# JokerYan/MS-GS

Measured on AMD Instinct MI355X. Metric: Mpixels/s fwd+bwd @1080p, 1M Gaussians; fraction of HBM roofline, higher is better.
Workload: dtype f32

## Files before the change

### ms-gs_amd/csrc/sort.hip

```cpp
#include "msgs_internal.h"

#include <algorithm>

namespace msgs {

namespace {

__device__ __forceinline__ uint32_t wave_inclusive_scan(uint32_t v, int lane) {
#pragma unroll
    for (int off = 1; off < 64; off <<= 1) {
        const uint32_t n = (uint32_t)__shfl_up((int)v, off);
        if (lane >= off) v += n;
    }
    return v;
}

__device__ __forceinline__ uint32_t block_exclusive_scan(uint32_t v, uint32_t* s_wave , uint32_t* total) {
    const int lane = threadIdx.x & 63, w = threadIdx.x >> 6;
    const uint32_t inc = wave_inclusive_scan(v, lane);
    if (lane == 63) s_wave[w] = inc;
    __syncthreads();
    uint32_t base = 0;
#pragma unroll
    for (int k = 0; k < 4; ++k) {
        const uint32_t t = s_wave[k];
        if (k < w) base += t;
    }
    *total = s_wave[0] + s_wave[1] + s_wave[2] + s_wave[3];
    __syncthreads();
    return base + inc - v;
}

__device__ __forceinline__ void scan_load_items(const uint32_t* in, int64_t base, int64_t n, uint32_t v[SCAN_ITEMS]) {
    static_assert(SCAN_ITEMS % 4 == 0, "uint4 runs");
    if (base + SCAN_ITEMS <= n && (reinterpret_cast<uintptr_t>(in + base) & 15) == 0) {
#pragma unroll
        for (int q = 0; q < SCAN_ITEMS / 4; ++q) {
            const uint4 a = *reinterpret_cast<const uint4*>(in + base + 4 * q);
            v[4 * q] = a.x; v[4 * q + 1] = a.y; v[4 * q + 2] = a.z; v[4 * q + 3] = a.w;
        }
    } else {
#pragma unroll
        for (int k = 0; k < SCAN_ITEMS; ++k) v[k] = base + k < n ? in[base + k] : 0u;
    }
}
__device__ __forceinline__ void scan_store_items(uint32_t* out, int64_t base, int64_t n, const uint32_t v[SCAN_ITEMS]) {
    if (base + SCAN_ITEMS <= n && (reinterpret_cast<uintptr_t>(out + base) & 15) == 0) {
#pragma unroll
        for (int q = 0; q < SCAN_ITEMS / 4; ++q)
            *reinterpret_cast<uint4*>(out + base + 4 * q) = make_uint4(v[4 * q], v[4 * q + 1], v[4 * q + 2], v[4 * q + 3]);
    } else {
#pragma unroll
        for (int k = 0; k < SCAN_ITEMS; ++k) if (base + k < n) out[base + k] = v[k];
    }
}

__global__ __launch_bounds__(SCAN_THREADS) void scan_reduce_kernel(const uint32_t* __restrict__ in,
                                                                   const uint32_t* __restrict__ gather,
                                                                   int64_t n, uint64_t* __restrict__ partials,
                                                                   uint32_t* __restrict__ staged,
                                                                   const uint32_t* __restrict__ n_ptr, uint32_t in_mask,
                                                                   uint32_t* __restrict__ side_out, uint32_t* __restrict__ side_flag) {
    __shared__ uint32_t s_wave[4];
    if (n_ptr) n = (int64_t)*n_ptr;
    if (side_flag && blockIdx.x == 0 && threadIdx.x == 0) *side_flag = side_out ? 1u : 0u;
    const int64_t base = (int64_t)blockIdx.x * SCAN_CHUNK + (int64_t)threadIdx.x * SCAN_ITEMS;
    uint32_t v[SCAN_ITEMS];
    if (gather) {
        uint32_t g[SCAN_ITEMS];
        scan_load_items(gather, base, n, g);
#pragma unroll
        for (int k = 0; k < SCAN_ITEMS; ++k) v[k] = base + k < n ? in[g[k]] : 0u;
        if (side_out) {
#pragma unroll
            for (int k = 0; k < SCAN_ITEMS; ++k) g[k] = v[k] >> TILE_COUNT_BITS;
            scan_store_items(side_out, base, n, g);
        }
#pragma unroll
        for (int k = 0; k < SCAN_ITEMS; ++k) v[k] &= in_mask;
        if (staged) scan_store_items(staged, base, n, v);
    } else {
        scan_load_items(in, base, n, v);
    }
    uint32_t sum = 0;
#pragma unroll
    for (int k = 0; k < SCAN_ITEMS; ++k) sum += v[k];
    uint32_t total;
    block_exclusive_scan(sum, s_wave, &total);
    if (threadIdx.x == 0) partials[blockIdx.x] = total;
}

__global__ __launch_bounds__(SCAN_THREADS) void scan_apply_fused_kernel(const uint32_t* in, uint32_t* out, int64_t n,
                                                                        const uint64_t* __restrict__ partials, int64_t nb,
                                                                        const uint32_t* __restrict__ n_ptr,
                                                                        uint64_t* __restrict__ total_out,
                                                                        uint64_t* __restrict__ status,
                                                                        volatile uint64_t* host, uint64_t ticket,
                                                                        uint32_t* __restrict__ clamped_total, uint64_t clamp,
                                                                        const uint32_t* __restrict__ extra,
                                                                        uint32_t* __restrict__ zero_word,
                                                                        uint32_t* __restrict__ overflow_flag) {
    __shared__ uint32_t s_wave[4];
    __shared__ uint64_t s_sum[4];
    if (n_ptr) n = (int64_t)*n_ptr;
    const int lane = threadIdx.x & 63, w = threadIdx.x >> 6;
    const int64_t chunk0 = (int64_t)blockIdx.x * SCAN_CHUNK;
    if (blockIdx.x != 0 && chunk0 >= n) return;
    const int64_t upto = blockIdx.x == 0 ? nb : (int64_t)blockIdx.x;
    uint64_t acc = 0;
    for (int64_t q = threadIdx.x; q < upto; q += SCAN_THREADS) acc += partials[q];
    for (int off = 32; off > 0; off >>= 1)
        acc += ((uint64_t)(uint32_t)__shfl_xor((int)(uint32_t)(acc >> 32), off) << 32) | (uint32_t)__shfl_xor((int)(uint32_t)acc, off);
    if (lane == 0) s_sum[w] = acc;
    __syncthreads();
    const uint64_t sum = s_sum[0] + s_sum[1] + s_sum[2] + s_sum[3];
    uint64_t base = sum;
    if (blockIdx.x == 0) {
        base = 0;
        if (threadIdx.x == 0) {
            if (total_out) *total_out = sum;
            if (zero_word) *zero_word = 0u;
            if (clamped_total) *clamped_total = (uint32_t)(sum < clamp ? sum : clamp);
            if (overflow_flag && sum > clamp) *overflow_flag = 1u;
            const uint64_t info = extra ? ((uint64_t)extra[0] | ((uint64_t)extra[1] << 32)) : 0ull;
            if (status) { status[0] = sum; status[1] = 0; status[2] = info; }
            if (host) {
                host[0] = sum;
                host[1] = 0;
                host[3] = info;
                __threadfence_system();
                host[2] = ticket;
            }
        }
        if (chunk0 >= n) return;
    }
    const int64_t tb = chunk0 + (int64_t)threadIdx.x * SCAN_ITEMS;
    uint32_t v[SCAN_ITEMS];
    scan_load_items(in, tb, n, v);
    uint32_t tsum = 0;
#pragma unroll
    for (int k = 0; k < SCAN_ITEMS; ++k) tsum += v[k];
    uint32_t total;
    uint32_t run = block_exclusive_scan(tsum, s_wave, &total) + (uint32_t)base;
#pragma unroll
    for (int k = 0; k < SCAN_ITEMS; ++k) {
        const uint32_t x = v[k];
        v[k] = run;
        run += x;
    }
    scan_store_items(out, tb, n, v);
}

template <int ITEMS = SORT_ITEMS>
__device__ __forceinline__ int64_t elem_index(int64_t chunk_base, int w, int r, int lane) {
    return chunk_base + (int64_t)w * (64 * ITEMS) + r * 64 + lane;
}

template <int ITEMS, bool DROP = false, typename KeyT = uint32_t>
__global__ __launch_bounds__(SORT_THREADS) void radix_hist_kernel(const KeyT* __restrict__ keys, int64_t n,
                                                                  int shift, uint32_t mask, int64_t nblocks,
                                                                  uint32_t* __restrict__ hist,
                                                                  uint32_t* __restrict__ gsum, int gsize, int ngroups,
                                                                  const uint32_t* __restrict__ n_ptr = nullptr) {
    __shared__ uint32_t s_hist[256];
    const int64_t chunk_base = (int64_t)blockIdx.x * (SORT_THREADS * ITEMS);
    if (n_ptr) {
        n = (int64_t)*n_ptr;
        if (chunk_base >= n) return;
    }
    s_hist[threadIdx.x] = 0;
    __syncthreads();
    const int lane = threadIdx.x & 63, w = threadIdx.x >> 6;
    constexpr int KPV = 16 / (int)sizeof(KeyT);
    if (ITEMS % KPV == 0 && chunk_base + (int64_t)SORT_THREADS * ITEMS <= n) {
        const uint4* kv = reinterpret_cast<const uint4*>(keys + chunk_base);
#pragma unroll
        for (int r = 0; r < ITEMS / KPV; ++r) {
            const uint4 v = kv[r * SORT_THREADS + threadIdx.x];
            const uint32_t w4[4] = {v.x, v.y, v.z, v.w};
#pragma unroll
            for (int j = 0; j < KPV; ++j) {
                const uint32_t k = sizeof(KeyT) == 4 ? w4[j] : ((w4[j >> 1] >> ((j & 1) * 16)) & 0xFFFFu);
                if (!DROP || k != 0xFFFFFFFFu) atomicAdd(&s_hist[(k >> shift) & mask], 1u);
            }
        }
    } else {
#pragma unroll
        for (int r = 0; r < ITEMS; ++r) {
            const int64_t i = elem_index<ITEMS>(chunk_base, w, r, lane);
            if (i < n) {
                const uint32_t k = (uint32_t)keys[i];
                if (!DROP || k != 0xFFFFFFFFu) atomicAdd(&s_hist[(k >> shift) & mask], 1u);
            }
        }
    }
    __syncthreads();
    const uint32_t c = s_hist[threadIdx.x];
    hist[(int64_t)blockIdx.x * 256 + threadIdx.x] = c;
    if (c) atomicAdd(&gsum[(int64_t)(blockIdx.x / gsize) * 256 + threadIdx.x], c);
}

__global__ __launch_bounds__(256) void group_scan_kernel(uint32_t* __restrict__ gsum, int ngroups,
                                                         uint32_t* __restrict__ hist, int gsize, int64_t nblocks,
                                                         const uint32_t* __restrict__ n_ptr, int chunk) {
    if (n_ptr) {
        const int64_t n = (int64_t)*n_ptr;
        nblocks = (n + chunk - 1) / chunk;
        ngroups = (int)((nblocks + gsize - 1) / gsize);
        if ((int)blockIdx.x > ngroups) return;
        if (nblocks == 0) return;
    }
    const int d = threadIdx.x;
    if ((int)blockIdx.x < ngroups) {
        const int64_t first = (int64_t)blockIdx.x * gsize;
        const int rows = (int)min((int64_t)gsize, nblocks - first);
        uint32_t* q = hist + first * 256 + d;
        uint32_t run = 0;
#pragma unroll 8
        for (int k = 0; k < rows; ++k) {
            const uint32_t v = q[(int64_t)k * 256];
            q[(int64_t)k * 256] = run;
            run += v;
        }
        return;
    }
    __shared__ uint32_t s_wv[4];
    uint32_t tot = 0;
#pragma unroll 8
    for (int k = 0; k < ngroups; ++k) tot += gsum[(int64_t)k * 256 + d];
    uint32_t dummy;
    uint32_t run = block_exclusive_scan(tot, s_wv, &dummy);
#pragma unroll 8
    for (int k = 0; k < ngroups; ++k) {
        uint32_t* q = &gsum[(int64_t)k * 256 + d];
        const uint32_t v = *q;
        *q = run;
        run += v;
    }
}

template <int ITEMS, bool DROP = false, typename KeyT = uint32_t>
__global__ __launch_bounds__(SORT_THREADS) void radix_scatter_kernel(const KeyT* __restrict__ keys_in,
                                                                     const uint32_t* __restrict__ vals_in,
                                                                     KeyT* __restrict__ keys_out,
                                                                     uint32_t* __restrict__ vals_out, int64_t n,
                                                                     int shift, uint32_t mask, int64_t nblocks,
                                                                     const uint32_t* __restrict__ hist_scanned,
                                                                     const uint32_t* __restrict__ gsum, int gsize,
                                                                     int ngroups, bool gsum_is_base = false,
                                                                     const uint32_t* __restrict__ n_ptr = nullptr,
                                                                     uint32_t* __restrict__ n_out = nullptr) {
    __shared__ uint32_t s_cnt[4][256];
    __shared__ uint32_t s_wave[4];
    const int lane = threadIdx.x & 63, w = threadIdx.x >> 6;
    const int64_t chunk_base = (int64_t)blockIdx.x * (SORT_THREADS * ITEMS);
    if (n_ptr) {
        n = (int64_t)*n_ptr;
        if (chunk_base >= n) return;
    }
#pragma unroll
    for (int k = 0; k < 4; ++k) s_cnt[k][threadIdx.x] = 0;
    __syncthreads();

    uint32_t key[ITEMS], val[ITEMS], rank[ITEMS];
    const uint64_t lt_mask = (1ull << lane) - 1ull;
#pragma unroll
    for (int r = 0; r < ITEMS; ++r) {
        const int64_t i = elem_index<ITEMS>(chunk_base, w, r, lane);
        key[r] = i < n ? (uint32_t)keys_in[i] : 0xFFFFFFFFu;
        const bool valid = i < n && (!DROP || key[r] != 0xFFFFFFFFu);
        val[r] = valid ? (vals_in ? vals_in[i] : (uint32_t)i) : 0u;
        const uint32_t d = (key[r] >> shift) & mask;
        uint64_t peers = __ballot(valid);
#pragma unroll
        for (int b = 0; b < 8; ++b) {
            const uint64_t m = __ballot((d >> b) & 1u);
            peers &= ((d >> b) & 1u) ? m : ~m;
        }
        const uint32_t prev = s_cnt[w][d];
        const uint32_t before = (uint32_t)__popcll(peers & lt_mask);
        rank[r] = prev + before;
        if (valid && before == 0) s_cnt[w][d] = prev + (uint32_t)__popcll(peers);
    }
    __syncthreads();
    uint32_t gbase;
    {
        const uint32_t d = threadIdx.x;
        if (gsum_is_base) {
            const int g = blockIdx.x / gsize;
            gbase = gsum[(int64_t)g * 256 + d] + hist_scanned[(int64_t)blockIdx.x * 256 + d];
        } else {
            const int g = blockIdx.x / gsize;
            uint32_t tot = 0, before = 0;
#pragma unroll 8
            for (int k = 0; k < ngroups; ++k) {
                const uint32_t v = gsum[(int64_t)k * 256 + d];
                tot += v;
                before += k < g ? v : 0u;
            }
            const int nin = (int)(blockIdx.x - (int64_t)g * gsize);
            const uint32_t* hrow = hist_scanned + ((int64_t)g * gsize) * 256 + d;
#pragma unroll 8
            for (int k = 0; k < nin; ++k) before += hrow[(int64_t)k * 256];
            uint32_t total;
            gbase = block_exclusive_scan(tot, s_wave, &total) + before;
            if (n_out && blockIdx.x == 0 && threadIdx.x == 0) *n_out = total;
        }
    }
    __shared__ uint32_t s_key[SORT_THREADS * ITEMS], s_val[SORT_THREADS * ITEMS], s_delta[256];
    uint32_t nkept;
    {
        const uint32_t d = threadIdx.x;
        uint32_t c[4], ltot = 0;
#pragma unroll
        for (int k = 0; k < 4; ++k) { c[k] = s_cnt[k][d]; ltot += c[k]; }
        const uint32_t lbase = block_exclusive_scan(ltot, s_wave, &nkept);
        uint32_t run = lbase;
#pragma unroll
        for (int k = 0; k < 4; ++k) { s_cnt[k][d] = run; run += c[k]; }
        s_delta[d] = gbase - lbase;
    }
    __syncthreads();
#pragma unroll
    for (int r = 0; r < ITEMS; ++r) {
        const int64_t i = elem_index<ITEMS>(chunk_base, w, r, lane);
        if (i < n && (!DROP || key[r] != 0xFFFFFFFFu)) {
            const uint32_t lp = s_cnt[w][(key[r] >> shift) & mask] + rank[r];
            s_key[lp] = key[r];
            s_val[lp] = val[r];
        }
    }
    __syncthreads();
    const int nvalid = DROP ? (int)nkept : (int)min((int64_t)(SORT_THREADS * ITEMS), n - chunk_base);
#pragma unroll
    for (int r = 0; r < ITEMS; ++r) {
        const int j = r * SORT_THREADS + threadIdx.x;
        if (j < nvalid) {
            const uint32_t k = s_key[j];
            const uint32_t pos = (uint32_t)j + s_delta[(k >> shift) & mask];
            keys_out[pos] = (KeyT)k;
            vals_out[pos] = s_val[j];
        }
    }
}

}

hipError_t exclusive_scan_u32(const uint32_t* in, const uint32_t* gather, uint32_t* out, int64_t n,
                              uint64_t* partials, uint64_t* total, hipStream_t s, uint64_t* status,
                              uint64_t* host_mapped, uint64_t ticket, const uint32_t* n_ptr, uint32_t* clamped_total,
                              uint64_t clamp, const uint32_t* extra, uint32_t* zero_word, uint32_t* overflow_flag,
                              uint32_t in_mask, uint32_t* side_out, uint32_t* side_flag) {
    if ((in_mask != 0xFFFFFFFFu || side_out) && gather == nullptr) return hipErrorInvalidValue;
    if (n <= 0) {
        hipLaunchKernelGGL(scan_apply_fused_kernel, dim3(1), dim3(SCAN_THREADS), 0, s, in, out, (int64_t)0,
                           (const uint64_t*)partials, (int64_t)0, (const uint32_t*)nullptr, total, status,
                           (volatile uint64_t*)host_mapped, ticket, clamped_total, clamp, extra, zero_word, overflow_flag);
        return hipGetLastError();
    }
    if (gather != nullptr && out == in) return hipErrorInvalidValue;
    const int64_t nb = scan_blocks(n);
    const bool stage = gather != nullptr;
    hipLaunchKernelGGL(scan_reduce_kernel, dim3((unsigned)nb), dim3(SCAN_THREADS), 0, s, in, gather, n, partials,
                       stage ? out : (uint32_t*)nullptr, n_ptr, in_mask, side_out, side_flag);
    hipLaunchKernelGGL(scan_apply_fused_kernel, dim3((unsigned)nb), dim3(SCAN_THREADS), 0, s,
                       stage ? (const uint32_t*)out : in, out, n, (const uint64_t*)partials, nb, n_ptr, total, status,
                       (volatile uint64_t*)host_mapped, ticket, clamped_total, clamp, extra, zero_word, overflow_flag);
    return hipGetLastError();
}

namespace {
__global__ __launch_bounds__(256) void zero_kernel(uint32_t* __restrict__ p, size_t n_words) {
    const size_t n4 = n_words >> 2;
    uint4* p4 = reinterpret_cast<uint4*>(p);
    for (size_t i = (size_t)blockIdx.x * blockDim.x + threadIdx.x; i < n4; i += (size_t)gridDim.x * blockDim.x)
        p4[i] = make_uint4(0u, 0u, 0u, 0u);
    if (blockIdx.x == 0 && threadIdx.x < (n_words & 3)) p[(n4 << 2) + threadIdx.x] = 0u;
}
}

hipError_t launch_zero(void* ptr, size_t bytes, hipStream_t s) {
    if (bytes == 0) return hipSuccess;
    if ((reinterpret_cast<uintptr_t>(ptr) & 15) || (bytes & 3)) return hipMemsetAsync(ptr, 0, bytes, s);
    const size_t words = bytes >> 2;
    size_t blocks = (words / 4 + 255) / 256;
    if (blocks < 1) blocks = 1;
    if (blocks > 2048) blocks = 2048;
    hipLaunchKernelGGL(zero_kernel, dim3((unsigned)blocks), dim3(256), 0, s, (uint32_t*)ptr, words);
    return hipGetLastError();
}

static int passes_for(int begin_bit, int end_bit) {
    const int passes = (end_bit - begin_bit + 7) / 8;
    return passes < 1 ? 1 : passes;
}
typedef SortGeom GroupGeom;

bool radix_sort_supports_device_count(int64_t n, int begin_bit, int end_bit) {
    return n > 0 && passes_for(begin_bit, end_bit) <= 4;
}

bool radix_sort_keys16_ok(int64_t n, int begin_bit, int end_bit) {
    return end_bit <= 16 && radix_sort_supports_device_count(n, begin_bit, end_bit);
}

bool radix_sort_zero_region(int64_t n, int begin_bit, int end_bit, char* scratch, uint32_t** ptr, size_t* words) {
    if (n <= 0) return false;
    const int passes = passes_for(begin_bit, end_bit);
    if (passes > 4) return false;
    const GroupGeom G(n);
    const SortScratch L(n);
    *ptr = reinterpret_cast<uint32_t*>(scratch + L.hist) + (size_t)256 * G.nb;
    *words = G.zero_words(passes);
    return true;
}

namespace {
__global__ void store_u32_kernel(uint32_t* p, uint32_t v) { *p = v; }

template <int ITEMS, typename KeyT>
void launch_pass(const KeyT* src_k, const uint32_t* src_v, KeyT* dst_k, uint32_t* dst_v, int64_t n, int shift, uint32_t mask,
                 const GroupGeom& G, uint32_t* hist, uint32_t* gs, bool drop, const uint32_t* n_ptr, uint32_t* n_out,
                 hipStream_t s) {
    const dim3 grid((unsigned)G.nb), block(SORT_THREADS);
    if (drop) {
        hipLaunchKernelGGL((radix_hist_kernel<ITEMS, true, KeyT>), grid, block, 0, s, src_k, n, shift, mask, G.nb, hist, gs, G.gsize,
                           G.ngroups, (const uint32_t*)nullptr);
        hipLaunchKernelGGL((radix_scatter_kernel<ITEMS, true, KeyT>), grid, block, 0, s, src_k, src_v, dst_k, dst_v, n, shift,
                           mask, G.nb, hist, gs, G.gsize, G.ngroups, false, (const uint32_t*)nullptr, n_out);
        return;
    }
    hipLaunchKernelGGL((radix_hist_kernel<ITEMS, false, KeyT>), grid, block, 0, s, src_k, n, shift, mask, G.nb, hist, gs, G.gsize,
                       G.ngroups, n_ptr);
    if (G.scanned)
        hipLaunchKernelGGL(group_scan_kernel, dim3((unsigned)G.ngroups + 1), dim3(256), 0, s, gs, G.ngroups, hist, G.gsize, G.nb, n_ptr,
                           SORT_THREADS * ITEMS);
    hipLaunchKernelGGL((radix_scatter_kernel<ITEMS, false, KeyT>), grid, block, 0, s, src_k, src_v, dst_k, dst_v, n, shift, mask,
                       G.nb, hist, gs, G.gsize, G.ngroups, G.scanned, n_ptr, (uint32_t*)nullptr);
}

template <typename KeyT>
hipError_t sort_passes(KeyT* keys_in, uint32_t* vals_in, KeyT* keys_out, uint32_t* vals_out, int64_t n, int passes,
                       int begin_bit, int end_bit, const GroupGeom& G, KeyT* keys_alt, uint32_t* vals_alt, uint32_t* hist,
                       uint32_t* gsum_all, bool compact, uint32_t* n_valid_dev, const uint32_t* n_dev, hipStream_t s) {
    const KeyT* src_k = keys_in;
    const uint32_t* src_v = vals_in;
    int next_shift = begin_bit;
    for (int p = 0; p < passes; ++p) {
        const int shift = next_shift;
        const int left = end_bit - shift;
        const int bits = (left + (passes - p) - 1) / (passes - p);
        next_shift = shift + bits;
        const uint32_t mask = bits >= 8 ? 0xFFu : ((1u << (bits > 0 ? bits : 1)) - 1u);
        const bool to_out = ((passes - 1 - p) % 2) == 0;
        KeyT* dst_k = to_out ? keys_out : keys_alt;
        uint32_t* dst_v = to_out ? vals_out : vals_alt;
        uint32_t* gs = gsum_all + (size_t)p * 256 * G.ngroups;
        const bool drop = compact && p == 0;
        const uint32_t* np = n_dev ? n_dev : (compact && p > 0 ? n_valid_dev : nullptr);
        uint32_t* no = drop ? n_valid_dev : nullptr;
        if (G.big) launch_pass<16, KeyT>(src_k, src_v, dst_k, dst_v, n, shift, mask, G, hist, gs, drop, np, no, s);
        else if (G.mid) launch_pass<8, KeyT>(src_k, src_v, dst_k, dst_v, n, shift, mask, G, hist, gs, drop, np, no, s);
        else launch_pass<SORT_ITEMS, KeyT>(src_k, src_v, dst_k, dst_v, n, shift, mask, G, hist, gs, drop, np, no, s);
        src_k = dst_k;
        src_v = dst_v;
    }
    return hipGetLastError();
}
}

hipError_t radix_sort_pairs(uint32_t* keys_in, uint32_t* vals_in, uint32_t* keys_out, uint32_t* vals_out,
                            int64_t n, int begin_bit, int end_bit, char* scratch, hipStream_t s, bool pre_zeroed,
                            uint32_t* n_valid_dev, const uint32_t* n_dev, bool keys16) {
    if (n <= 0) {
        if (n_valid_dev) hipLaunchKernelGGL(store_u32_kernel, dim3(1), dim3(1), 0, s, n_valid_dev, 0u);
        return hipSuccess;
    }
    const int passes = passes_for(begin_bit, end_bit);
    if (passes > 4) return hipErrorInvalidValue;
    const SortScratch L(n);
    uint32_t* keys_alt = reinterpret_cast<uint32_t*>(scratch + L.keys_alt);
    uint32_t* vals_alt = reinterpret_cast<uint32_t*>(scratch + L.vals_alt);
    uint32_t* hist = reinterpret_cast<uint32_t*>(scratch + L.hist);
    const GroupGeom G(n);
    uint32_t* gsum_all = hist + (size_t)256 * G.nb;
    if (!pre_zeroed) {
        hipError_t e = launch_zero(gsum_all, sizeof(uint32_t) * G.zero_words(passes), s);
        if (e != hipSuccess) return e;
    }
    if (keys16) {
        if (n_valid_dev || end_bit > 16) return hipErrorInvalidValue;
        return sort_passes<uint16_t>(reinterpret_cast<uint16_t*>(keys_in), vals_in, reinterpret_cast<uint16_t*>(keys_out), vals_out,
                                     n, passes, begin_bit, end_bit, G, reinterpret_cast<uint16_t*>(keys_alt), vals_alt, hist,
                                     gsum_all, false, nullptr, n_dev, s);
    }
    const bool compact = n_valid_dev != nullptr && !G.scanned;
    if (n_valid_dev && !compact) hipLaunchKernelGGL(store_u32_kernel, dim3(1), dim3(1), 0, s, n_valid_dev, (uint32_t)n);
    return sort_passes<uint32_t>(keys_in, vals_in, keys_out, vals_out, n, passes, begin_bit, end_bit, G, keys_alt, vals_alt, hist,
                                 gsum_all, compact, n_valid_dev, n_dev, s);
}

}
```

Baseline: 1988.

## Split radix scatter prefix-table reads across waves and batch key/value loads

The scatter kernel's per-block prefix computation used to have every thread walk all group-sum and in-group histogram rows serially. It now spreads those rows across the four waves, reading 16-byte vectors in batches of twelve, and combines the partial sums through shared memory borrowed from the reorder buffer. Key and value loads are issued up front, using clamped indices instead of per-element bounds checks, and are specialised on whether values are present. Launch bounds now request higher occupancy, and the histogram kernel also preloads its vector keys before the atomics. The intent is to hide global latency in a sort pass, at the cost of more registers and shared-buffer aliasing.

```diff
diff --git a/ms-gs_amd/csrc/sort.hip b/ms-gs_amd/csrc/sort.hip
--- a/ms-gs_amd/csrc/sort.hip
+++ b/ms-gs_amd/csrc/sort.hip
@@ -174,9 +174,12 @@
     constexpr int KPV = 16 / (int)sizeof(KeyT);
     if (ITEMS % KPV == 0 && chunk_base + (int64_t)SORT_THREADS * ITEMS <= n) {
         const uint4* kv = reinterpret_cast<const uint4*>(keys + chunk_base);
+        uint4 kq[ITEMS >= KPV ? ITEMS / KPV : 1];
+#pragma unroll
+        for (int r = 0; r < ITEMS / KPV; ++r) kq[r] = kv[r * SORT_THREADS + threadIdx.x];
 #pragma unroll
         for (int r = 0; r < ITEMS / KPV; ++r) {
-            const uint4 v = kv[r * SORT_THREADS + threadIdx.x];
+            const uint4 v = kq[r];
             const uint32_t w4[4] = {v.x, v.y, v.z, v.w};
 #pragma unroll
             for (int j = 0; j < KPV; ++j) {
@@ -239,8 +242,162 @@
     }
 }
 
+constexpr int SORT_TABLE_BATCH = 12;
+__device__ __forceinline__ void table_rows_load(const uint32_t* __restrict__ gsum, const uint32_t* __restrict__ hist_group,
+                                                int ngroups, int nrows, int first, int lane, uint4 v[SORT_TABLE_BATCH]) {
+#pragma unroll
+    for (int j = 0; j < SORT_TABLE_BATCH; ++j) {
+        const int row = min(first + 4 * j, nrows - 1);
+        const uintptr_t p = row < ngroups ? reinterpret_cast<uintptr_t>(gsum) + (uintptr_t)row * 1024
+                                          : reinterpret_cast<uintptr_t>(hist_group) + (uintptr_t)(row - ngroups) * 1024;
+        typedef uint32_t u32x4 __attribute__((ext_vector_type(4)));
+        const u32x4 q = reinterpret_cast<const __attribute__((address_space(1))) u32x4*>(p)[lane];
+        v[j] = make_uint4(q.x, q.y, q.z, q.w);
+    }
+}
+__device__ __forceinline__ void table_rows_add(const uint4 v[SORT_TABLE_BATCH], int ngroups, int nrows, int g, int first,
+                                               uint4& tot, uint4& bef) {
+#pragma unroll
+    for (int j = 0; j < SORT_TABLE_BATCH; ++j) {
+        const int row = first + 4 * j;
+        const uint32_t mt = row < ngroups ? 0xFFFFFFFFu : 0u;
+        const uint32_t mb = row < nrows && (row >= ngroups || row < g) ? 0xFFFFFFFFu : 0u;
+        tot.x += v[j].x & mt; tot.y += v[j].y & mt; tot.z += v[j].z & mt; tot.w += v[j].w & mt;
+        bef.x += v[j].x & mb; bef.y += v[j].y & mb; bef.z += v[j].z & mb; bef.w += v[j].w & mb;
+        asm volatile("" : "+v"(tot.x), "+v"(tot.y), "+v"(tot.z), "+v"(tot.w), "+v"(bef.x), "+v"(bef.y), "+v"(bef.z), "+v"(bef.w));
+    }
+}
+
+template <int ITEMS, bool DROP, typename KeyT, bool HAS_VALS>
+__device__ __forceinline__ void radix_scatter_block(const KeyT* __restrict__ keys_in, const uint32_t* __restrict__ vals_in,
+                                                    KeyT* __restrict__ keys_out, uint32_t* __restrict__ vals_out, int64_t n,
+                                                    int shift, uint32_t mask, const uint32_t* __restrict__ hist_scanned,
+                                                    const uint32_t* __restrict__ gsum, int gsize, int ngroups, bool gsum_is_base,
+                                                    uint32_t* __restrict__ n_out, uint32_t (*s_cnt)[256], uint32_t* s_wave,
+                                                    uint32_t* s_kv, uint32_t* s_delta) {
+    uint32_t* const s_key = s_kv;
+    uint32_t* const s_val = s_kv + SORT_THREADS * ITEMS;
+    const int lane = threadIdx.x & 63, w = threadIdx.x >> 6;
+    const int wu = __builtin_amdgcn_readfirstlane(w);
+    const int64_t chunk_base = (int64_t)blockIdx.x * (SORT_THREADS * ITEMS);
+    const int g = blockIdx.x / gsize;
+    const int nrows = ngroups + (int)(blockIdx.x - (int64_t)g * gsize);
+    const uint32_t* hist_group = hist_scanned + ((int64_t)g * gsize) * 256;
+    uint32_t base_g = 0, base_h = 0;
+    uint4 trow[SORT_TABLE_BATCH];
+    uint4 tot = make_uint4(0u, 0u, 0u, 0u), bef = make_uint4(0u, 0u, 0u, 0u);
+    int first = wu;
+    if (gsum_is_base) {
+        base_g = gsum[(int64_t)g * 256 + threadIdx.x];
+        base_h = hist_scanned[(int64_t)blockIdx.x * 256 + threadIdx.x];
+    } else {
+#pragma clang loop unroll(disable) vectorize(disable) interleave(disable)
+        for (; first + 4 * SORT_TABLE_BATCH < nrows; first += 4 * SORT_TABLE_BATCH) {
+            table_rows_load(gsum, hist_group, ngroups, nrows, first, lane, trow);
+            table_rows_add(trow, ngroups, nrows, g, first, tot, bef);
+        }
+        table_rows_load(gsum, hist_group, ngroups, nrows, first, lane, trow);
+    }
+    const uint32_t off0 = (uint32_t)(w * (64 * ITEMS) + lane);
+    const uint32_t last = (uint32_t)min((int64_t)(SORT_THREADS * ITEMS), n - chunk_base) - 1u;
+    uint32_t key[ITEMS], val[ITEMS], rank[ITEMS];
+    const KeyT* kb = keys_in + chunk_base;
+#pragma unroll
+    for (int r = 0; r < ITEMS; ++r) key[r] = (uint32_t)kb[min(off0 + r * 64, last)];
+#pragma unroll
+    for (int k = 0; k < 4; ++k) s_cnt[k][threadIdx.x] = 0;
+    if (gsum_is_base) {
+        s_kv[threadIdx.x] = base_g + base_h;
+    } else {
+        table_rows_add(trow, ngroups, nrows, g, first, tot, bef);
+        uint4* const s_part = reinterpret_cast<uint4*>(s_kv) + wu * 128 + lane;
+        s_part[0] = tot;
+        s_part[64] = bef;
+    }
+    __builtin_amdgcn_sched_barrier(0);
+    if (HAS_VALS) {
+        const uint32_t* vb = vals_in + chunk_base;
+#pragma unroll
+        for (int r = 0; r < ITEMS; ++r) val[r] = vb[min(off0 + r * 64, last)];
+    } else {
+#pragma unroll
+        for (int r = 0; r < ITEMS; ++r) val[r] = (uint32_t)chunk_base + off0 + r * 64;
+    }
+    __syncthreads();
+
+    const uint64_t lt_mask = (1ull << lane) - 1ull;
+#pragma unroll
+    for (int r = 0; r < ITEMS; ++r) {
+        const bool valid = off0 + r * 64 <= last && (!DROP || key[r] != 0xFFFFFFFFu);
+        const uint32_t d = (key[r] >> shift) & mask;
+        uint64_t peers = __ballot(valid);
+#pragma unroll
+        for (int b = 0; b < 8; ++b) {
+            const uint64_t m = __ballot((d >> b) & 1u);
+            peers &= ((d >> b) & 1u) ? m : ~m;
+        }
+        const uint32_t prev = s_cnt[w][d];
+        const uint32_t before = (uint32_t)__popcll(peers & lt_mask);
+        rank[r] = prev + before;
+        if (valid && before == 0) s_cnt[w][d] = prev + (uint32_t)__popcll(peers);
+    }
+    __syncthreads();
+    uint32_t gbase;
+    {
+        const uint32_t d = threadIdx.x;
+        if (gsum_is_base) {
+            gbase = s_kv[d];
+        } else {
+            uint32_t tot = 0, before = 0;
+#pragma unroll
+            for (int k = 0; k < 4; ++k) {
+                tot += s_kv[(2 * k) * 256 + d];
+                before += s_kv[(2 * k + 1) * 256 + d];
+            }
+            uint32_t total;
+            gbase = block_exclusive_scan(tot, s_wave, &total) + before;
+            if (n_out && blockIdx.x == 0 && threadIdx.x == 0) *n_out = total;
+        }
+    }
+    uint32_t nkept;
+    {
+        const uint32_t d = threadIdx.x;
+        uint32_t c[4], ltot = 0;
+#pragma unroll
+        for (int k = 0; k < 4; ++k) { c[k] = s_cnt[k][d]; ltot += c[k]; }
+        const uint32_t lbase = block_exclusive_scan(ltot, s_wave, &nkept);
+        uint32_t run = lbase;
+#pragma unroll
+        for (int k = 0; k < 4; ++k) { s_cnt[k][d] = run; run += c[k]; }
+        s_delta[d] = gbase - lbase;
+    }
+    __syncthreads();
+#pragma unroll
+    for (int r = 0; r < ITEMS; ++r) {
+        uint32_t k = key[r];
+        asm volatile("" : "+v"(k));
+        if (off0 + r * 64 <= last && (!DROP || k != 0xFFFFFFFFu)) {
+            const uint32_t lp = s_cnt[w][(k >> shift) & mask] + rank[r];
+            s_key[lp] = k;
+            s_val[lp] = val[r];
+        }
+    }
+    __syncthreads();
+    const int nvalid = DROP ? (int)nkept : (int)last + 1;
+#pragma unroll
+    for (int r = 0; r < ITEMS; ++r) {
+        const int j = r * SORT_THREADS + threadIdx.x;
+        if (j < nvalid) {
+            const uint32_t k = s_key[j];
+            const uint32_t pos = (uint32_t)j + s_delta[(k >> shift) & mask];
+            keys_out[pos] = (KeyT)k;
+            vals_out[pos] = s_val[j];
+        }
+    }
+}
+
 template <int ITEMS, bool DROP = false, typename KeyT = uint32_t>
-__global__ __launch_bounds__(SORT_THREADS) void radix_scatter_kernel(const KeyT* __restrict__ keys_in,
+__global__ __launch_bounds__(SORT_THREADS, 4) void radix_scatter_kernel(const KeyT* __restrict__ keys_in,
                                                                      const uint32_t* __restrict__ vals_in,
                                                                      KeyT* __restrict__ keys_out,
                                                                      uint32_t* __restrict__ vals_out, int64_t n,
@@ -250,98 +407,21 @@
                                                                      int ngroups, bool gsum_is_base = false,
                                                                      const uint32_t* __restrict__ n_ptr = nullptr,
                                                                      uint32_t* __restrict__ n_out = nullptr) {
+    static_assert(ITEMS >= 4, "the table partials borrow 2048 words of the reorder buffers");
     __shared__ uint32_t s_cnt[4][256];
     __shared__ uint32_t s_wave[4];
-    const int lane = threadIdx.x & 63, w = threadIdx.x >> 6;
-    const int64_t chunk_base = (int64_t)blockIdx.x * (SORT_THREADS * ITEMS);
+    __shared__ __attribute__((aligned(16))) uint32_t s_kv[2 * SORT_THREADS * ITEMS];
+    __shared__ uint32_t s_delta[256];
     if (n_ptr) {
         n = (int64_t)*n_ptr;
-        if (chunk_base >= n) return;
-    }
-#pragma unroll
-    for (int k = 0; k < 4; ++k) s_cnt[k][threadIdx.x] = 0;
-    __syncthreads();
-
-    uint32_t key[ITEMS], val[ITEMS], rank[ITEMS];
-    const uint64_t lt_mask = (1ull << lane) - 1ull;
-#pragma unroll
-    for (int r = 0; r < ITEMS; ++r) {
-        const int64_t i = elem_index<ITEMS>(chunk_base, w, r, lane);
-        key[r] = i < n ? (uint32_t)keys_in[i] : 0xFFFFFFFFu;
-        const bool valid = i < n && (!DROP || key[r] != 0xFFFFFFFFu);
-        val[r] = valid ? (vals_in ? vals_in[i] : (uint32_t)i) : 0u;
-        const uint32_t d = (key[r] >> shift) & mask;
-        uint64_t peers = __ballot(valid);
-#pragma unroll
-        for (int b = 0; b < 8; ++b) {
-            const uint64_t m = __ballot((d >> b) & 1u);
-            peers &= ((d >> b) & 1u) ? m : ~m;
-        }
-        const uint32_t prev = s_cnt[w][d];
-        const uint32_t before = (uint32_t)__popcll(peers & lt_mask);
-        rank[r] = prev + before;
-        if (valid && before == 0) s_cnt[w][d] = prev + (uint32_t)__popcll(peers);
-    }
-    __syncthreads();
-    uint32_t gbase;
-    {
-        const uint32_t d = threadIdx.x;
-        if (gsum_is_base) {
-            const int g = blockIdx.x / gsize;
-            gbase = gsum[(int64_t)g * 256 + d] + hist_scanned[(int64_t)blockIdx.x * 256 + d];
-        } else {
-            const int g = blockIdx.x / gsize;
-            uint32_t tot = 0, before = 0;
-#pragma unroll 8
-            for (int k = 0; k < ngroups; ++k) {
-                const uint32_t v = gsum[(int64_t)k * 256 + d];
-                tot += v;
-                before += k < g ? v : 0u;
-            }
-            const int nin = (int)(blockIdx.x - (int64_t)g * gsize);
-            const uint32_t* hrow = hist_scanned + ((int64_t)g * gsize) * 256 + d;
-#pragma unroll 8
-            for (int k = 0; k < nin; ++k) before += hrow[(int64_t)k * 256];
-            uint32_t total;
-            gbase = block_exclusive_scan(tot, s_wave, &total) + before;
-            if (n_out && blockIdx.x == 0 && threadIdx.x == 0) *n_out = total;
-        }
-    }
-    __shared__ uint32_t s_key[SORT_THREADS * ITEMS], s_val[SORT_THREADS * ITEMS], s_delta[256];
-    uint32_t nkept;
-    {
-        const uint32_t d = threadIdx.x;
-        uint32_t c[4], ltot = 0;
-#pragma unroll
-        for (int k = 0; k < 4; ++k) { c[k] = s_cnt[k][d]; ltot += c[k]; }
-        const uint32_t lbase = block_exclusive_scan(ltot, s_wave, &nkept);
-        uint32_t run = lbase;
-#pragma unroll
-        for (int k = 0; k < 4; ++k) { s_cnt[k][d] = run; run += c[k]; }
-        s_delta[d] = gbase - lbase;
-    }
-    __syncthreads();
-#pragma unroll
-    for (int r = 0; r < ITEMS; ++r) {
-        const int64_t i = elem_index<ITEMS>(chunk_base, w, r, lane);
-        if (i < n && (!DROP || key[r] != 0xFFFFFFFFu)) {
-            const uint32_t lp = s_cnt[w][(key[r] >> shift) & mask] + rank[r];
-            s_key[lp] = key[r];
-            s_val[lp] = val[r];
-        }
-    }
-    __syncthreads();
-    const int nvalid = DROP ? (int)nkept : (int)min((int64_t)(SORT_THREADS * ITEMS), n - chunk_base);
-#pragma unroll
-    for (int r = 0; r < ITEMS; ++r) {
-        const int j = r * SORT_THREADS + threadIdx.x;
-        if (j < nvalid) {
-            const uint32_t k = s_key[j];
-            const uint32_t pos = (uint32_t)j + s_delta[(k >> shift) & mask];
-            keys_out[pos] = (KeyT)k;
-            vals_out[pos] = s_val[j];
-        }
-    }
+        if ((int64_t)blockIdx.x * (SORT_THREADS * ITEMS) >= n) return;
+    }
+    if (vals_in)
+        radix_scatter_block<ITEMS, DROP, KeyT, true>(keys_in, vals_in, keys_out, vals_out, n, shift, mask, hist_scanned, gsum, gsize,
+                                                     ngroups, gsum_is_base, n_out, s_cnt, s_wave, s_kv, s_delta);
+    else
+        radix_scatter_block<ITEMS, DROP, KeyT, false>(keys_in, vals_in, keys_out, vals_out, n, shift, mask, hist_scanned, gsum, gsize,
+                                                      ngroups, gsum_is_base, n_out, s_cnt, s_wave, s_kv, s_delta);
 }
 
 }
```

Result: no change. 2010, median of 6 (+1.1%).
